# zju-vipa/ProtoPFormer

Measured on AMD Instinct MI355X. Metric: images/sec train step, deit_small+2000 protos, bs256, 1/2/4/8 MI355X, higher is better.
Workload: dtype bf16; 1 GPU; deit_small_patch16_224, synthetic 224x224, 2000x384 prototypes, 200 classes, k=81, batch 256/GPU (BASELINE.json configs[2]), train step = fwd+CE+PPC+bwd+allreduce+AdamW+EMA, DropPath 0.1; blocks after the token reservation run compacted on the 1+k reserved rows (equal to the masked full-length blocks to bf16 rounding); bf16 backbone: the reserved tokens differ from the fp32 reference's in ~2-3 % o; global_batch=256, parallelism=dp1

## Files before the change

protopformer_amd/csrc/gemm_bf16.hip:

```cpp
#include "ppf_common.h"
#include "ppf_hip.h"
#include "gemm_common.h"
#include "gemm_layout.h"
#include <cstdlib>
#include <type_traits>

namespace {
using namespace ppfg;

constexpr int BM = 128, BN = 128, NTHREADS = 256;
constexpr int TILE_BYTES = BM * BK * 2;
constexpr int STAGE_LD = 68;
constexpr int STAGE_BYTES = 4 * 32 * STAGE_LD * 4;


__device__ __forceinline__ int lds_off_mode0(int r, int c16) { return lds_row_off(r, c16); }

typedef uint32_t u32x4 __attribute__((ext_vector_type(4)));

template <bool T, int ROWS, int NTHR = NTHREADS>
struct TileIO {
    static constexpr int NLD = ROWS * 8 / NTHR;
    static constexpr int RPP = NTHR / 8;
    static constexpr int CPR = ROWS / 8;
    static constexpr int KPP = NTHR / CPR;
    static __device__ __forceinline__ unsigned gload(u32x4 (&reg)[NLD], const bf16_t* __restrict__ X, int ld, int R, int row0,
                                                     int k0, int kend, int tid, int kpad) {
        unsigned mask = 0;
        if constexpr (!T) {
            const int c16 = tid & 7, rb = tid >> 3;
            const bool kok = kpad ? (k0 + c16 * 8) < kend : (k0 + c16 * 8 + 8) <= kend;
            const int kk = kok ? k0 + c16 * 8 : 0;
#pragma unroll
            for (int i = 0; i < NLD; ++i) {
                const int r = row0 + rb + RPP * i;
                const bf16_t* src = X + (size_t)min(r, R - 1) * ld + kk;
                reg[i] = *reinterpret_cast<const u32x4*>(src);
                mask |= (kok && r < R) ? (1u << i) : 0u;
            }
        } else {
            const int c16 = tid % CPR, kb = tid / CPR;
            const int col = row0 + c16 * 8;
            const bool cok = kpad ? col < R : (col + 8) <= R;
            const int cc = cok ? col : 0;
#pragma unroll
            for (int i = 0; i < NLD; ++i) {
                const int kc = k0 + kb + KPP * i;
                const bf16_t* src = X + (size_t)min(kc, kend - 1) * ld + cc;
                reg[i] = *reinterpret_cast<const u32x4*>(src);
                mask |= (cok && kc < kend) ? (1u << i) : 0u;
            }
        }
        return mask;
    }
    static __device__ __forceinline__ void sstore(const u32x4 (&reg)[NLD], unsigned mask, unsigned char* tile, int tid) {
        const u32x4 zero = {0u, 0u, 0u, 0u};
        if constexpr (!T) {
            const int c16 = tid & 7, rb = tid >> 3;
#pragma unroll
            for (int i = 0; i < NLD; ++i)
                *reinterpret_cast<u32x4*>(tile + lds_off_mode0(rb + RPP * i, c16)) = ((mask >> i) & 1u) ? reg[i] : zero;
        } else {
            const int c16 = tid % CPR, kb = tid / CPR;
#pragma unroll
            for (int i = 0; i < NLD; ++i)
                *reinterpret_cast<u32x4*>(tile + lds_off_mode1<ROWS>(kb + KPP * i, c16 * 8)) = ((mask >> i) & 1u) ? reg[i] : zero;
        }
    }
    static __device__ __forceinline__ bf16x8 frag(const unsigned char* tile, int rbase, int ks, int lane) {
        if constexpr (!T) {
            return *reinterpret_cast<const bf16x8*>(tile + lds_off_mode0(rbase + (lane & 31), ks * 2 + (lane >> 5)));
        } else {
            typedef __attribute__((address_space(3))) bf16x4 lds_bf16x4;
            const int s = lane & 15, g16 = (lane >> 4) & 1, h = lane >> 5;
            const int col = rbase + 16 * g16 + 4 * (s & 3);
            const int kc = ks * 16 + 8 * h + (s >> 2);
            bf16x4 lo = __builtin_amdgcn_ds_read_tr16_b64_v4bf16((lds_bf16x4*)(tile + lds_off_mode1<ROWS>(kc, col)));
            bf16x4 hi = __builtin_amdgcn_ds_read_tr16_b64_v4bf16((lds_bf16x4*)(tile + lds_off_mode1<ROWS>(kc + 4, col)));
            return __builtin_shufflevector(lo, hi, 0, 1, 2, 3, 4, 5, 6, 7);
        }
    }
};


template <int EPI>
__device__ __forceinline__ void epilogue_rows(const GemmParams& p, const float* stage, int mbase, int nbase, int lane) {
    if (EpiWide<EPI>::value && ((p.ldc | p.ldaux) & 7) == 0) {
        const int col = (lane & 7) * 8;
        const int n = nbase + col;
        if (n + 8 <= p.N) {
            const EpiCols8 cc = epi_load_cols8<EPI>(p, n, true);
            EpiRow8 rr[4];
#pragma unroll
            for (int pass = 0; pass < 4; ++pass) {
                const int m = mbase + pass * 8 + (lane >> 3);
                rr[pass] = epi_load_row8<EPI>(p, m, n, m < p.M);
            }
#pragma unroll
            for (int pass = 0; pass < 4; ++pass) {
                const int r = pass * 8 + (lane >> 3);
                const int m = mbase + r;
                const float4 a = *reinterpret_cast<const float4*>(stage + r * STAGE_LD + col);
                const float4 b = *reinterpret_cast<const float4*>(stage + r * STAGE_LD + col + 4);
                if (m < p.M) epi_store8<EPI>(p, m, n, a, b, cc, rr[pass]);
            }
        } else if (n < p.N) {
            const EpiCols cc = epi_load_cols<EPI>(p, n, true);
#pragma unroll
            for (int pass = 0; pass < 4; ++pass) {
                const int r = pass * 8 + (lane >> 3);
                const int m = mbase + r;
                if (m < p.M) {
                    const EpiRow rr = epi_load_row<EPI>(p, m, n, true);
                    const float4 v = *reinterpret_cast<const float4*>(stage + r * STAGE_LD + col);
                    epi_store<EPI>(p, m, n, v.x, v.y, v.z, v.w, cc, rr);
                }
            }
        }
    } else {
        const int col = (lane & 15) * 4;
        const int n = nbase + col;
        const EpiCols cc = epi_load_cols<EPI>(p, n, n < p.N);
        EpiRow rr[8];
#pragma unroll
        for (int pass = 0; pass < 8; ++pass) {
            const int m = mbase + pass * 4 + (lane >> 4);
            rr[pass] = epi_load_row<EPI>(p, m, n, m < p.M && n < p.N);
        }
#pragma unroll
        for (int pass = 0; pass < 8; ++pass) {
            const int r = pass * 4 + (lane >> 4);
            const int m = mbase + r;
            const float4 v = *reinterpret_cast<const float4*>(stage + r * STAGE_LD + col);
            if (m < p.M && n < p.N) epi_store<EPI>(p, m, n, v.x, v.y, v.z, v.w, cc, rr[pass]);
        }
    }
}

template <int EPI, int MT>
__device__ __forceinline__ void strip_epilogue(const GemmParams& p, const f32x16 (&acc)[2][MT], int mi, unsigned char* smem, int wave, int lane,
                                               int mbase, int nbase) {
    const int h = lane >> 5;
    float* stage = reinterpret_cast<float*>(smem) + wave * (32 * STAGE_LD);
#pragma unroll
    for (int ni = 0; ni < 2; ++ni)
#pragma unroll
        for (int g = 0; g < 4; ++g)
            *reinterpret_cast<float4*>(stage + (lane & 31) * STAGE_LD + 32 * ni + 8 * g + 4 * h) =
                make_float4(acc[ni][mi][4 * g], acc[ni][mi][4 * g + 1], acc[ni][mi][4 * g + 2], acc[ni][mi][4 * g + 3]);
    __builtin_amdgcn_wave_barrier();
    epilogue_rows<EPI>(p, stage, mbase, nbase, lane);
    __builtin_amdgcn_wave_barrier();
}

__device__ __forceinline__ void store_partial_colsum(const GemmParams& p, int m, float v) {
    p.ws[p.zslice * ((size_t)p.M * p.N + (size_t)p.cs_parts * p.M) + (size_t)p.M * p.N + m] = v;
}

template <bool TA, bool TB, int EPI, bool COLSUM>
__global__ __launch_bounds__(NTHREADS, 3) void gemm_kernel(const GemmParams p_) {
    constexpr int PD = 1, MT = 2;
    extern __shared__ __attribute__((aligned(16))) unsigned char smem[];
    constexpr int TBM = 64 * MT;
    constexpr int A_BYTES = TBM * BK * 2;
    using IOA = TileIO<TA, TBM>;
    using IOB = TileIO<TB, BN>;
    const int tid = threadIdx.x, lane = tid & 63, wave = tid >> 6;
    const int wm = (wave & 1) * (32 * MT), wn = (wave >> 1) * 64;

    const int tiles_n = (p_.N + BN - 1) / BN;
    const int tiles = tiles_n * ((p_.M + TBM - 1) / TBM);
    const int vid_all = xcd_remap(blockIdx.x, gridDim.x);
    const int zslice = vid_all / tiles, vid = vid_all - zslice * tiles;
    const int m0 = (vid / tiles_n) * TBM, n0 = (vid % tiles_n) * BN;
    GemmParams p = p_;
    p.zslice = zslice;
    if (gridDim.y > 1) {
        const int bo = blockIdx.y / p.batch_inner, bi = blockIdx.y % p.batch_inner;
        p.A += bo * p.sa_o + bi * p.sa_i;
        p.B += bo * p.sb_o + bi * p.sb_i;
        const long long co = bo * p.sc_o + bi * p.sc_i;
        p.C = (EPI == EPI_BF16) ? (void*)(reinterpret_cast<bf16_t*>(p.C) + co) : (void*)(reinterpret_cast<float*>(p.C) + co);
    }

    const auto [kbeg, kend] = k_slice(p.K, p.nsplit, zslice);
    if (kbeg >= kend) return;
    const int nk = (kend - kbeg + BK - 1) / BK;

    u32x4 ra[PD][IOA::NLD], rb[PD][IOB::NLD];
    unsigned ma[PD], mb[PD];
    f32x16 acc[2][MT];
#pragma unroll
    for (int i = 0; i < 2; ++i)
#pragma unroll
        for (int j = 0; j < MT; ++j)
#pragma unroll
            for (int r = 0; r < 16; ++r) acc[i][j][r] = 0.f;
    f32x16 accs[MT];
    if constexpr (COLSUM) {
#pragma unroll
        for (int j = 0; j < MT; ++j)
#pragma unroll
            for (int r = 0; r < 16; ++r) accs[j][r] = 0.f;
    }
    const bool do_colsum = COLSUM && p.colsum != nullptr && n0 == 0 && wn == 0;
    unsigned char* tA = smem;
    unsigned char* tB = smem + A_BYTES;

#pragma unroll
    for (int st = 0; st < PD; ++st) {
        const int k0 = min(kbeg + st * BK, kbeg + (nk - 1) * BK);
        ma[st] = IOA::gload(ra[st], p.A, p.lda, p.M, m0, k0, kend, tid, p.kpad);
        mb[st] = IOB::gload(rb[st], p.B, p.ldb, p.N, n0, k0, kend, tid, p.kpad);
    }
    IOA::sstore(ra[0], ma[0], tA, tid);
    IOB::sstore(rb[0], mb[0], tB, tid);
    __syncthreads();

    for (int kt0 = 0; kt0 < nk; kt0 += PD) {
#pragma unroll
        for (int u = 0; u < PD; ++u) {
            const int kt = kt0 + u;
            if (kt >= nk) break;
            {
                const int k0 = kbeg + min(kt + PD, nk - 1) * BK;
                ma[u] = IOA::gload(ra[u], p.A, p.lda, p.M, m0, k0, kend, tid, p.kpad);
                mb[u] = IOB::gload(rb[u], p.B, p.ldb, p.N, n0, k0, kend, tid, p.kpad);
            }
#pragma unroll
            for (int ks = 0; ks < BK / 16; ++ks) {
                bf16x8 fa[MT], fb[2];
#pragma unroll
                for (int i = 0; i < MT; ++i) fa[i] = IOA::frag(tA, wm + 32 * i, ks, lane);
#pragma unroll
                for (int i = 0; i < 2; ++i) fb[i] = IOB::frag(tB, wn + 32 * i, ks, lane);
#pragma unroll
                for (int ni = 0; ni < 2; ++ni)
#pragma unroll
                    for (int mi = 0; mi < MT; ++mi)
                        acc[ni][mi] = __builtin_amdgcn_mfma_f32_32x32x16_bf16(fb[ni], fa[mi], acc[ni][mi], 0, 0, 0);
                if constexpr (COLSUM) {
                    if (do_colsum) {
                        bf16x8 ones;
#pragma unroll
                        for (int e = 0; e < 8; ++e) ones[e] = (__bf16)1.0f;
#pragma unroll
                        for (int mi = 0; mi < MT; ++mi)
                            accs[mi] = __builtin_amdgcn_mfma_f32_32x32x16_bf16(ones, fa[mi], accs[mi], 0, 0, 0);
                    }
                }
            }
            __syncthreads();
            if (kt + 1 < nk) {
                IOA::sstore(ra[(u + 1) % PD], ma[(u + 1) % PD], tA, tid);
                IOB::sstore(rb[(u + 1) % PD], mb[(u + 1) % PD], tB, tid);
            }
            __syncthreads();
        }
    }

#pragma unroll
    for (int mi = 0; mi < MT; ++mi) {
        strip_epilogue<EPI>(p, acc, mi, smem, wave, lane, m0 + wm + 32 * mi, n0 + wn);
        if constexpr (COLSUM) {
            const int m = m0 + wm + 32 * mi + (lane & 31);
            if (do_colsum && (lane >> 5) == 0 && m < p.M) {
                if constexpr (EPI == EPI_PARTIAL) store_partial_colsum(p, m, accs[mi][0]);
                else unsafeAtomicAdd(p.colsum + m, accs[mi][0]);
            }
        }
    }
}

#ifndef WG8_ISSUE_REGIONS
#define WG8_ISSUE_REGIONS 3
#endif
template <bool COLSUM>
__device__ __forceinline__ void wgrad8_mma(const bf16x8 (&fa)[2], const bf16x8 (&fb)[2], f32x16 (&acc)[2][2], f32x16 (&accs)[2], bool do_colsum) {
#pragma unroll
    for (int ni = 0; ni < 2; ++ni)
#pragma unroll
        for (int mi = 0; mi < 2; ++mi) acc[ni][mi] = __builtin_amdgcn_mfma_f32_32x32x16_bf16(fb[ni], fa[mi], acc[ni][mi], 0, 0, 0);
    if constexpr (COLSUM) {
        if (do_colsum) {
            bf16x8 ones;
#pragma unroll
            for (int e = 0; e < 8; ++e) ones[e] = (__bf16)1.0f;
#pragma unroll
            for (int mi = 0; mi < 2; ++mi) accs[mi] = __builtin_amdgcn_mfma_f32_32x32x16_bf16(ones, fa[mi], accs[mi], 0, 0, 0);
        }
    }
}

template <int WMW, int WNW, bool COLSUM, bool DMA>
__global__ __launch_bounds__(64 * WMW * WNW, 1) void wgrad8_kernel(const GemmParams p_) {
    extern __shared__ __attribute__((aligned(16))) unsigned char smem[];
    constexpr int NTHR = 64 * WMW * WNW, TBM = 64 * WMW, TBN = 64 * WNW;
    using IOA = TileIO<true, TBM, NTHR>;
    using IOB = TileIO<true, TBN, NTHR>;
    const int tid = threadIdx.x, lane = tid & 63;
    const int wave = __builtin_amdgcn_readfirstlane(tid >> 6);
    const int wm = (wave % WMW) * 64, wn = (wave / WMW) * 64;
    const int tiles_n = (p_.N + TBN - 1) / TBN;
    const int tiles = tiles_n * ((p_.M + TBM - 1) / TBM);
    const int vid_all = xcd_remap(blockIdx.x, gridDim.x);
    const int zslice = vid_all / tiles, vid = vid_all - zslice * tiles;
    const int m0 = (vid / tiles_n) * TBM, n0 = (vid % tiles_n) * TBN;
    GemmParams p = p_;
    p.zslice = zslice;
    const auto [kbeg, kend] = k_slice(p.K, p.nsplit, zslice);
    if (kbeg >= kend) return;
    const int nk = (kend - kbeg + BK - 1) / BK;

    f32x16 acc[2][2];
#pragma unroll
    for (int i = 0; i < 2; ++i)
#pragma unroll
        for (int j = 0; j < 2; ++j)
#pragma unroll
            for (int r = 0; r < 16; ++r) acc[i][j][r] = 0.f;
    f32x16 accs[2];
    if constexpr (COLSUM) {
#pragma unroll
        for (int j = 0; j < 2; ++j)
#pragma unroll
            for (int r = 0; r < 16; ++r) accs[j][r] = 0.f;
    }
    const bool do_colsum = COLSUM && p.colsum != nullptr && n0 == 0 && wn == 0;
    constexpr int A_BYTES = TBM * BK * 2;
    if constexpr (!DMA) {
        u32x4 ra[IOA::NLD], rb[IOB::NLD];
        unsigned ma, mb;
        unsigned char* tA = smem;
        unsigned char* tB = smem + A_BYTES;
        ma = IOA::gload(ra, p.A, p.lda, p.M, m0, kbeg, kend, tid, 0);
        mb = IOB::gload(rb, p.B, p.ldb, p.N, n0, kbeg, kend, tid, 0);
        IOA::sstore(ra, ma, tA, tid);
        IOB::sstore(rb, mb, tB, tid);
        __syncthreads();
        for (int kt = 0; kt < nk; ++kt) {
            {
                const int k0 = kbeg + min(kt + 1, nk - 1) * BK;
                ma = IOA::gload(ra, p.A, p.lda, p.M, m0, k0, kend, tid, 0);
                mb = IOB::gload(rb, p.B, p.ldb, p.N, n0, k0, kend, tid, 0);
            }
#pragma unroll
            for (int ks = 0; ks < BK / 16; ++ks) {
                bf16x8 fa[2], fb[2];
#pragma unroll
                for (int i = 0; i < 2; ++i) fa[i] = IOA::frag(tA, wm + 32 * i, ks, lane);
#pragma unroll
                for (int i = 0; i < 2; ++i) fb[i] = IOB::frag(tB, wn + 32 * i, ks, lane);
                wgrad8_mma<COLSUM>(fa, fb, acc, accs, do_colsum);
            }
            __syncthreads();
            if (kt + 1 < nk) {
                IOA::sstore(ra, ma, tA, tid);
                IOB::sstore(rb, mb, tB, tid);
            }
            __syncthreads();
        }
    } else {
        constexpr int NPA = TBM / 8, NPB = TBN / 8, PPW = (NPA + NPB) / 8;
        static_assert(NTHR == 512 && A_BYTES + TBN * BK * 2 == WG8_SLOT_BYTES && NPA % 8 == 0, "ring slot layout");
        const unsigned offA = (unsigned)(wgrad_dma_src(wgrad_dma_piece<TBM>(wave, lane), 0, p.lda, m0, p.M) * 2);
        const unsigned offB = (unsigned)(wgrad_dma_src(wgrad_dma_piece<TBN>(wave, lane), 0, p.ldb, n0, p.N) * 2);
        const size_t stepA = (size_t)p.lda * (BK * 2), stepB = (size_t)p.ldb * (BK * 2);
        const size_t pieceA = (size_t)p.lda * (4096 / TBM * 2), pieceB = (size_t)p.ldb * (4096 / TBN * 2);
        const unsigned char* gA = reinterpret_cast<const unsigned char*>(p.A) + (size_t)kbeg * p.lda * 2;
        const unsigned char* gB = reinterpret_cast<const unsigned char*>(p.B) + (size_t)kbeg * p.ldb * 2;
        const uint32_t ring = __builtin_amdgcn_readfirstlane(lds_offset_of(smem)) + wave * 1024;
        auto issue = [&](int i, uint32_t dst) __attribute__((always_inline)) {
            if (8 * i < NPA) lds_dma16_hidden(gA + i * pieceA + offA, dst + 8192 * i);
            else lds_dma16_hidden(gB + (i - NPA / 8) * pieceB + offB, dst + 8192 * i);
        };

        auto tile = [&](const unsigned char* st, uint32_t nxt, auto issue_tag) __attribute__((always_inline)) {
            constexpr bool ISSUE = decltype(issue_tag)::value;
            constexpr int NKS = BK / 16, NRI = WG8_ISSUE_REGIONS;
            const unsigned char* tA = st;
            const unsigned char* tB = st + A_BYTES;
            bf16x8 fa[2][2], fb[2][2];
#pragma unroll
            for (int i = 0; i < 2; ++i) fa[0][i] = IOA::frag(tA, wm + 32 * i, 0, lane);
#pragma unroll
            for (int i = 0; i < 2; ++i) fb[0][i] = IOB::frag(tB, wn + 32 * i, 0, lane);
#pragma unroll
            for (int ks = 0; ks < NKS; ++ks) {
                __builtin_amdgcn_sched_barrier(0);
                if constexpr (ISSUE) {
                    if (ks < NRI) {
#pragma unroll
                        for (int k = ks * PPW / NRI; k < (ks + 1) * PPW / NRI; ++k) issue(k, nxt);
                    }
                }
                if (ks + 1 < NKS) {
#pragma unroll
                    for (int i = 0; i < 2; ++i) fa[(ks + 1) & 1][i] = IOA::frag(tA, wm + 32 * i, ks + 1, lane);
#pragma unroll
                    for (int i = 0; i < 2; ++i) fb[(ks + 1) & 1][i] = IOB::frag(tB, wn + 32 * i, ks + 1, lane);
                }
                wgrad8_mma<COLSUM>(fa[ks & 1], fb[ks & 1], acc, accs, do_colsum);
            }
            __builtin_amdgcn_sched_barrier(0);
        };

#pragma unroll
        for (int i = 0; i < PPW; ++i) issue(i, ring);
        int slot = 0;
        for (int kt = 0; kt + 1 < nk; ++kt) {
            asm volatile("s_waitcnt vmcnt(0)" ::: "memory");
            __builtin_amdgcn_s_barrier();
            gA += stepA;
            gB += stepB;
            tile(smem + slot * WG8_SLOT_BYTES, ring + (slot ^ 1) * WG8_SLOT_BYTES, std::true_type());
            slot ^= 1;
        }
        asm volatile("s_waitcnt vmcnt(0)" ::: "memory");
        __builtin_amdgcn_s_barrier();
        tile(smem + slot * WG8_SLOT_BYTES, 0u, std::false_type());
        __syncthreads();
    }
#pragma unroll
    for (int mi = 0; mi < 2; ++mi) {
        strip_epilogue<EPI_PARTIAL>(p, acc, mi, smem, wave, lane, m0 + wm + 32 * mi, n0 + wn);
        if constexpr (COLSUM) {
            const int m = m0 + wm + 32 * mi + (lane & 31);
            if (do_colsum && (lane >> 5) == 0 && m < p.M) store_partial_colsum(p, m, accs[mi][0]);
        }
    }
}

int g_wgrad_path = 0;
#ifndef PPF_WGRAD_DMA_DEFAULT
#define PPF_WGRAD_DMA_DEFAULT 1
#endif
bool wgrad8_dma(const GemmParams& p) {
    if (p.K % BK != 0 || g_wgrad_path == 1) return false;
    return g_wgrad_path == 2 || PPF_WGRAD_DMA_DEFAULT;
}

template <int WMW, int WNW>
int launch_wgrad8(const GemmParams& p, int splitk, hipStream_t stream) {
    constexpr int NTHR = 64 * WMW * WNW, TBM = 64 * WMW, TBN = 64 * WNW;
    constexpr int opnd = (TBM + TBN) * BK * 2, strips = (NTHR / 64) * 32 * STAGE_LD * 4;
    constexpr int lds = opnd > strips ? opnd : strips;
    static_assert(strips <= WG8_RING_BYTES, "the epilogue strips reuse the dead ring");
    const int tiles = ((p.M + TBM - 1) / TBM) * ((p.N + TBN - 1) / TBN);
    if (wgrad8_dma(p)) return ppf_launch<wgrad8_kernel<WMW, WNW, true, true>>(dim3(tiles * splitk), dim3(NTHR), WG8_RING_BYTES, stream, "wgrad8 (dma)", p);
    return ppf_launch<wgrad8_kernel<WMW, WNW, true, false>>(dim3(tiles * splitk), dim3(NTHR), lds, stream, "wgrad8", p);
}

typedef __attribute__((address_space(3))) void g4_lds_t;
typedef const __attribute__((address_space(1))) void g4_gbl_t;

template <int NLA>
struct DirectLds {
    unsigned offA[NLA], offB[4];
    const unsigned char *gA, *gB;
    __device__ __forceinline__ DirectLds(const GemmParams& p, int m0, int n0, int tid)
        : gA(reinterpret_cast<const unsigned char*>(p.A)), gB(reinterpret_cast<const unsigned char*>(p.B)) {
        const int rb = tid >> 3, ch = (tid & 7) ^ lds_swz(rb);
#pragma unroll
        for (int i = 0; i < NLA; ++i) offA[i] = ((unsigned)min(m0 + rb + 32 * i, p.M - 1) * (unsigned)p.lda + ch * 8) * 2u;
#pragma unroll
        for (int i = 0; i < 4; ++i) offB[i] = ((unsigned)min(n0 + rb + 32 * i, p.N - 1) * (unsigned)p.ldb + ch * 8) * 2u;
    }
    __device__ __forceinline__ void load(int kt, unsigned char* tA, unsigned char* tB, int wave) const {
        const unsigned char* ka = gA + (size_t)kt * (BK * 2);
        const unsigned char* kb = gB + (size_t)kt * (BK * 2);
#pragma unroll
        for (int i = 0; i < NLA; ++i)
            __builtin_amdgcn_global_load_lds((g4_gbl_t*)(ka + offA[i]), (g4_lds_t*)(tA + i * 4096 + wave * 1024), 16, 0, 0);
#pragma unroll
        for (int i = 0; i < 4; ++i)
            __builtin_amdgcn_global_load_lds((g4_gbl_t*)(kb + offB[i]), (g4_lds_t*)(tB + i * 4096 + wave * 1024), 16, 0, 0);
        asm volatile("s_waitcnt vmcnt(0)" ::: "memory");
        __syncthreads();
    }
};

template <int EPI>
__global__ __launch_bounds__(NTHREADS, 4) void gemm128g_kernel(const GemmParams p) {
    extern __shared__ __attribute__((aligned(16))) unsigned char smem[];
    using IO = TileIO<false, 128>;
    const int tid = threadIdx.x, lane = tid & 63;
    const int wave = __builtin_amdgcn_readfirstlane(tid >> 6);
    const int wm = (wave & 1) * 64, wn = (wave >> 1) * 64;
    const int tiles_n = (p.N + BN - 1) / BN;
    const int vid = xcd_remap(blockIdx.x, gridDim.x);
    const int m0 = (vid / tiles_n) * BM, n0 = (vid % tiles_n) * BN;
    unsigned char* tA = smem;
    unsigned char* tB = smem + TILE_BYTES;
    const DirectLds<BM / 32> dl(p, m0, n0, tid);
    f32x16 acc[2][2];
#pragma unroll
    for (int i = 0; i < 2; ++i)
#pragma unroll
        for (int j = 0; j < 2; ++j)
#pragma unroll
            for (int r = 0; r < 16; ++r) acc[i][j][r] = 0.f;

    const int nk = p.K / BK;
    for (int kt = 0; kt < nk; ++kt) {
        if (kt > 0) __syncthreads();
        dl.load(kt, tA, tB, wave);
#pragma unroll
        for (int ks = 0; ks < BK / 16; ++ks) {
            bf16x8 fa[2], fb[2];
#pragma unroll
            for (int i = 0; i < 2; ++i) fa[i] = IO::frag(tA, wm + 32 * i, ks, lane);
#pragma unroll
            for (int i = 0; i < 2; ++i) fb[i] = IO::frag(tB, wn + 32 * i, ks, lane);
#pragma unroll
            for (int ni = 0; ni < 2; ++ni)
#pragma unroll
                for (int mi = 0; mi < 2; ++mi)
                    acc[ni][mi] = __builtin_amdgcn_mfma_f32_32x32x16_bf16(fb[ni], fa[mi], acc[ni][mi], 0, 0, 0);
        }
    }
    __syncthreads();
#pragma unroll
    for (int mi = 0; mi < 2; ++mi) strip_epilogue<EPI>(p, acc, mi, smem, wave, lane, m0 + wm + 32 * mi, n0 + wn);
}

template <int EPI>
int launch_g4(const GemmParams& p, hipStream_t stream) {
    constexpr int lds = 2 * TILE_BYTES > STAGE_BYTES ? 2 * TILE_BYTES : STAGE_BYTES;
    const int tiles = ((p.M + BM - 1) / BM) * ((p.N + BN - 1) / BN);
    return ppf_launch<gemm128g_kernel<EPI>>(dim3(tiles), dim3(NTHREADS), lds, stream, "gemm128g", p);
}

constexpr int G224_ROWS = 224, G224_MT = 7, G224_LD = 36;
__global__ __launch_bounds__(NTHREADS, 3) void gemm224g_kernel(const GemmParams p) {
    extern __shared__ __attribute__((aligned(16))) unsigned char smem[];
    using IO = TileIO<false, 128>;
    const int tid = threadIdx.x, lane = tid & 63;
    const int wave = __builtin_amdgcn_readfirstlane(tid >> 6);
    const int wn = wave * 32;
    const int tiles_n = (p.N + BN - 1) / BN;
    const int vid = xcd_remap(blockIdx.x, gridDim.x);
    const int m0 = (vid / tiles_n) * G224_ROWS, n0 = (vid % tiles_n) * BN;
    unsigned char* tA = smem;
    unsigned char* tB = smem + G224_ROWS * BK * 2;
    const DirectLds<G224_MT> dl(p, m0, n0, tid);
    f32x16 acc[G224_MT];
#pragma unroll
    for (int j = 0; j < G224_MT; ++j)
#pragma unroll
        for (int r = 0; r < 16; ++r) acc[j][r] = 0.f;
    const int nk = p.K / BK;
    for (int kt = 0; kt < nk; ++kt) {
        if (kt > 0) __syncthreads();
        dl.load(kt, tA, tB, wave);
#pragma unroll
        for (int ks = 0; ks < BK / 16; ++ks) {
            const bf16x8 fb = IO::frag(tB, wn, ks, lane);
#pragma unroll
            for (int mi = 0; mi < G224_MT; ++mi)
                acc[mi] = __builtin_amdgcn_mfma_f32_32x32x16_bf16(fb, IO::frag(tA, 32 * mi, ks, lane), acc[mi], 0, 0, 0);
        }
    }
    __syncthreads();
    const int h = lane >> 5;
    float* stage = reinterpret_cast<float*>(smem) + wave * (32 * G224_LD);
    bf16_t* C = reinterpret_cast<bf16_t*>(p.C);
#pragma unroll
    for (int mi = 0; mi < G224_MT; ++mi) {
#pragma unroll
        for (int g = 0; g < 4; ++g)
            *reinterpret_cast<float4*>(stage + (lane & 31) * G224_LD + 8 * g + 4 * h) =
                make_float4(acc[mi][4 * g], acc[mi][4 * g + 1], acc[mi][4 * g + 2], acc[mi][4 * g + 3]);
        __builtin_amdgcn_fence(__ATOMIC_RELEASE, "wavefront");
        __builtin_amdgcn_wave_barrier();
#pragma unroll
        for (int pass = 0; pass < 2; ++pass) {
            const int r = pass * 16 + (lane >> 2), col = (lane & 3) * 8;
            const int m = m0 + 32 * mi + r, n = n0 + wn + col;
            const float4 a = *reinterpret_cast<const float4*>(stage + r * G224_LD + col);
            const float4 b = *reinterpret_cast<const float4*>(stage + r * G224_LD + col + 4);
            if (m < p.M && n < p.N)
                *reinterpret_cast<uint4*>(C + (size_t)m * p.ldc + n) = make_uint4(pack_bf16x2(a.x * p.alpha, a.y * p.alpha), pack_bf16x2(a.z * p.alpha, a.w * p.alpha),
                                                                                 pack_bf16x2(b.x * p.alpha, b.y * p.alpha), pack_bf16x2(b.z * p.alpha, b.w * p.alpha));
        }
        __builtin_amdgcn_fence(__ATOMIC_RELEASE, "wavefront");
        __builtin_amdgcn_wave_barrier();
    }
}

bool g4_eligible(const GemmParams& p);
int g_force_g224 = 0;
bool g224_eligible(const GemmParams& p, int epi) {
    if (epi != EPI_BF16 || p.bias != nullptr || p.kpad || p.K % BK != 0 || p.N % 8 != 0 || (p.ldc & 7) != 0) return false;
    if ((long long)p.M * p.lda >= (1ll << 30) || (long long)p.N * p.ldb >= (1ll << 30)) return false;
    if (g_force_g224) return true;
    if (p.K < 768) return false;
    const int cus = ppf_cu_count();
    const long long tn = (p.N + BN - 1) / BN;
    const long long t128 = (long long)((p.M + BM - 1) / BM) * tn, t224 = (long long)((p.M + G224_ROWS - 1) / G224_ROWS) * tn;
    const int per128 = g4_eligible(p) ? 4 : 3;
    auto cost = [](long long tiles, long long slots, int rows, int per) {
        const long long full = tiles / slots, rest = tiles - full * slots;
        double c = (double)full * rows * per;
        if (rest) c += rows * per * (4 * rest >= slots ? 1.0 : 0.5);
        return c;
    };
    return t128 >= (long long)per128 * cus && cost(t224, 3ll * cus, G224_ROWS, 3) < 0.97 * cost(t128, (long long)per128 * cus, BM, per128);
}
int launch_g224(const GemmParams& p, hipStream_t stream) {
    constexpr int lds = G224_ROWS * BK * 2 + TILE_BYTES;
    const int tiles = ((p.M + G224_ROWS - 1) / G224_ROWS) * ((p.N + BN - 1) / BN);
    return ppf_launch<gemm224g_kernel>(dim3(tiles), dim3(NTHREADS), lds, stream, "gemm224g", p);
}

bool g4_eligible(const GemmParams& p) {
    return p.K % BK == 0 && p.K <= 512 && p.N >= 512 && !p.kpad && (long long)p.M * p.lda < (1ll << 30) &&
           (long long)p.N * p.ldb < (1ll << 30) && (long long)((p.M + BM - 1) / BM) * ((p.N + BN - 1) / BN) >= 512;
}

template <bool TA, bool TB, int EPI, bool COLSUM>
int launch(const GemmParams& p, int splitk, hipStream_t stream, int nbatch = 1) {
    const int tiles = ((p.M + BM - 1) / BM) * ((p.N + BN - 1) / BN);
    constexpr int lds = 2 * TILE_BYTES > STAGE_BYTES ? 2 * TILE_BYTES : STAGE_BYTES;
    GemmParams q = p;
    q.nsplit = splitk;
    return ppf_launch<gemm_kernel<TA, TB, EPI, COLSUM>>(dim3(tiles * splitk, nbatch, 1), dim3(NTHREADS), lds, stream, "gemm", q);
}

__global__ __launch_bounds__(256) void splitk_reduce_kernel(const float* __restrict__ ws, float* __restrict__ C, float* __restrict__ colsum,
                                                            int M, int N, int ldc, int nsplit, int cs_parts) {
    const size_t mn = (size_t)M * N, slice = mn + (colsum ? (size_t)cs_parts * M : 0);
    const size_t total4 = mn / 4;
    const size_t i = (size_t)blockIdx.x * 256 + threadIdx.x;
    if (i < total4) {
        const float* p = ws + i * 4;
        float4 acc = make_float4(0.f, 0.f, 0.f, 0.f);
        for (int z0 = 0; z0 < nsplit; z0 += 16) {
            float4 v[16];
#pragma unroll
            for (int u = 0; u < 16; ++u) {
                const int z = min(z0 + u, nsplit - 1);
                v[u] = *reinterpret_cast<const float4*>(p + (size_t)z * slice);
            }
#pragma unroll
            for (int u = 0; u < 16; ++u)
                if (z0 + u < nsplit) { acc.x += v[u].x; acc.y += v[u].y; acc.z += v[u].z; acc.w += v[u].w; }
        }
        const size_t e = i * 4, m = e / N, n = e - m * N;
        float4* dst = reinterpret_cast<float4*>(C + m * ldc + n);
        const float4 c = *dst;
        *dst = make_float4(c.x + acc.x, c.y + acc.y, c.z + acc.z, c.w + acc.w);
    } else if (colsum && i < total4 + (size_t)M) {
        const size_t m = i - total4;
        float a = 0.f;
        for (int z = 0; z < nsplit; ++z)
            for (int q = 0; q < cs_parts; ++q) a += ws[(size_t)z * slice + mn + (size_t)q * M + m];
        colsum[m] += a;
    }
}

PpfEventPool g_probe;
bool g_probe_on = false;

constexpr size_t PPF_GEMM_COUNTER_BYTES = 16384;


template <int... EPIS, class F>
bool dispatch_epi(int epi, int& rc, F&& f) {
    return ((epi == EPIS && (rc = f(std::integral_constant<int, EPIS>()), true)) || ...);
}

}

extern "C" {

int ppf_gemm_test_force_g224(int force) { g_force_g224 = force != 0; return 0; }

int ppf_gemm_test_wgrad_path(int path) {
    PPF_CHECK_ARG(path >= 0 && path <= 2, PPF_ERR_ARG, "ppf_gemm_test_wgrad_path: path must be 0, 1 or 2 (got %d)", path);
    g_wgrad_path = path;
    return 0;
}

size_t ppf_gemm_workspace_bytes(int M, int N, int K) {
    return PPF_GEMM_COUNTER_BYTES + (size_t)pick_splitk(M, N, K) * ((size_t)M * N + M) * sizeof(float);
}

int ppf_gemm_bf16(const void* A, const void* B, void* C, int M, int N, int K, int lda, int ldb, int ldc, int trans_a,
                  int trans_b, int epi, const float* bias, const float* res, int ldres, const float* rowscale,
                  int rows_per_group, const float* colscale, const void* aux_in, void* aux_out, int ldaux, float* colsum,
                  float alpha, void* workspace, size_t workspace_bytes, hipStream_t stream) {
    PPF_CHECK_ARG(M > 0 && N > 0 && K > 0, PPF_ERR_SHAPE, "ppf_gemm_bf16: bad shape M=%d N=%d K=%d", M, N, K);
    PPF_CHECK_ARG((lda % 8) == 0 && (ldb % 8) == 0 && (ldc % 4) == 0 && (N % 4) == 0, PPF_ERR_ALIGN,
                  "ppf_gemm_bf16: lda/ldb must be multiples of 8, ldc and N of 4 (lda=%d ldb=%d ldc=%d N=%d)", lda, ldb, ldc, N);
    PPF_CHECK_ARG(trans_a ? (M % 8 == 0) : (K % 8 == 0), PPF_ERR_ALIGN, "ppf_gemm_bf16: A inner extent must be a multiple of 8");
    PPF_CHECK_ARG(trans_b ? (N % 8 == 0) : (K % 8 == 0), PPF_ERR_ALIGN, "ppf_gemm_bf16: B inner extent must be a multiple of 8");
    PPF_CHECK_ARG((((uintptr_t)A | (uintptr_t)B | (uintptr_t)C) & 15) == 0, PPF_ERR_ALIGN, "ppf_gemm_bf16: pointers must be 16-byte aligned");
    PPF_CHECK_ARG(!(trans_a && !trans_b), PPF_ERR_ARG, "ppf_gemm_bf16: (trans_a=1, trans_b=0) is not instantiated");
    PPF_CHECK_ARG((((uintptr_t)aux_in | (uintptr_t)aux_out | (uintptr_t)res) & 15) == 0 && (ldaux % 4) == 0 && (ldres % 4) == 0, PPF_ERR_ALIGN,
                  "ppf_gemm_bf16: aux / residual pointers must be 16-byte aligned, ldaux and ldres multiples of 4 (the epilogues use 8/16-byte accesses)");
    GemmParams p;
    p.A = (const bf16_t*)A; p.B = (const bf16_t*)B; p.C = C; p.M = M; p.N = N; p.K = K; p.lda = lda; p.ldb = ldb; p.ldc = ldc;
    p.bias = bias; p.res = res; p.ldres = ldres; p.rowscale = rowscale; p.rows_per_group = rows_per_group > 0 ? rows_per_group : 1;
    p.colscale = colscale; p.aux_in = (const bf16_t*)aux_in; p.aux_out = (bf16_t*)aux_out; p.ldaux = ldaux; p.colsum = colsum; p.alpha = alpha; p.ws = nullptr;
    p.batch_inner = 1; p.sa_o = p.sa_i = p.sb_o = p.sb_i = p.sc_o = p.sc_i = 0; p.kpad = 0; p.cs_parts = 1; p.nsplit = 1;
    if (epi == EPI_RESID) PPF_CHECK_ARG(res != nullptr, PPF_ERR_ARG, "ppf_gemm_bf16: epi=4 needs a residual");
    if (epi == EPI_GELU) PPF_CHECK_ARG(aux_out != nullptr, PPF_ERR_ARG, "ppf_gemm_bf16: epi=2 needs aux_out");
    if (epi == EPI_DGELU) PPF_CHECK_ARG(aux_in != nullptr, PPF_ERR_ARG, "ppf_gemm_bf16: epi=5 needs aux_in");
    int rc;
    if (!trans_a && !trans_b) {
        if (g224_eligible(p, epi)) return launch_g224(p, stream);
        const auto g4 = [&](auto e) { return launch_g4<decltype(e)::value>(p, stream); };
        const auto nt = [&](auto e) { return launch<false, false, decltype(e)::value, false>(p, 1, stream); };
        if (g4_eligible(p) && dispatch_epi<EPI_BF16, EPI_GELU, EPI_RESID, EPI_DGELU>(epi, rc, g4)) return rc;
        if (dispatch_epi<EPI_BF16, EPI_F32, EPI_GELU, EPI_SIGMOID_F32, EPI_RESID, EPI_DGELU>(epi, rc, nt)) return rc;
    } else if (!trans_a && trans_b) {
        const auto nn = [&](auto e) { return launch<false, true, decltype(e)::value, false>(p, 1, stream); };
        if (dispatch_epi<EPI_BF16, EPI_F32, EPI_DGELU>(epi, rc, nn)) return rc;
    } else if (epi == EPI_ATOMIC) {
        const int ns = pick_splitk(M, N, K);
        const size_t need = PPF_GEMM_COUNTER_BYTES + (size_t)ns * ((size_t)M * N + M) * sizeof(float);
        if (workspace == nullptr || workspace_bytes < need || ns == 1) return launch<true, true, EPI_ATOMIC, true>(p, ns, stream);
        p.ws = (float*)((unsigned char*)workspace + PPF_GEMM_COUNTER_BYTES);
        p.cs_parts = 1;
        p.nsplit = ns;
        hipEvent_t e1 = nullptr;
        if (g_probe_on) {
            const auto ev = g_probe.acquire();
            (void)hipEventRecord(ev.first, stream);
            e1 = ev.second;
        }
        const bool wide = (M < N ? M : N) >= 320;
        if (wide && M >= 512 && M >= N && (M % 256 == 0 || M >= 1024)) rc = launch_wgrad8<4, 2>(p, ns, stream);
        else if (wide && N >= 512 && (N % 256 == 0 || N >= 1024)) rc = launch_wgrad8<2, 4>(p, ns, stream);
        else rc = launch<true, true, EPI_PARTIAL, true>(p, ns, stream);
        if (rc) return rc;
        if (e1) {
            (void)hipEventRecord(e1, stream);
            g_probe.flops += 2.0 * M * N * (double)K;
            g_probe.bytes += 2.0 * ((double)M * K + (double)N * K) + 4.0 * M * N;
        }
        const size_t work = (size_t)M * N / 4 + (colsum ? M : 0);
        const int grid = (int)((work + 255) / 256);
        hipLaunchKernelGGL(splitk_reduce_kernel, dim3(grid), dim3(256), 0, stream, p.ws, (float*)C, colsum, M, N, ldc, ns, p.cs_parts);
        PPF_LAUNCH_CHECK();
        return 0;
    } else if (epi == EPI_F32) {
        return launch<true, true, EPI_F32, false>(p, 1, stream);
    }
    ppf_set_error("ppf_gemm_bf16: combination trans_a=%d trans_b=%d epi=%d not instantiated", trans_a, trans_b, epi);
    return PPF_ERR_ARG;
}

int ppf_gemm_probe(int enable) {
    if (enable == 1) g_probe.reset();
    if (enable == 2) g_probe.destroy();
    g_probe_on = enable == 1;
    return 0;
}
int ppf_gemm_probe_read(double* ms_total, int64_t* launches, double* flops, double* bytes) {
    return g_probe.sum_ms("ppf_gemm_probe_read", ms_total, launches, flops, bytes);
}

int ppf_gemm_bf16_batched(const void* A, const void* B, void* C, int M, int N, int K, int lda, int ldb, int ldc, int trans_a, int trans_b,
                          int out_f32, float alpha, int batch_outer, int batch_inner, int64_t sa_o, int64_t sa_i, int64_t sb_o, int64_t sb_i,
                          int64_t sc_o, int64_t sc_i, int kpad, hipStream_t stream) {
    PPF_CHECK_ARG(M > 0 && N > 0 && K > 0 && batch_outer > 0 && batch_inner > 0, PPF_ERR_SHAPE, "ppf_gemm_bf16_batched: bad shape");
    PPF_CHECK_ARG((lda % 8) == 0 && (ldb % 8) == 0 && (ldc % 4) == 0 && (N % 4) == 0, PPF_ERR_ALIGN, "ppf_gemm_bf16_batched: ld alignment");
    PPF_CHECK_ARG(kpad || (trans_a ? (M % 8 == 0) : (K % 8 == 0)), PPF_ERR_ALIGN, "ppf_gemm_bf16_batched: A inner extent must be a multiple of 8");
    PPF_CHECK_ARG(kpad || (trans_b ? (N % 8 == 0) : (K % 8 == 0)), PPF_ERR_ALIGN, "ppf_gemm_bf16_batched: B inner extent must be a multiple of 8");
    PPF_CHECK_ARG(((sa_o | sa_i | sb_o | sb_i) % 8) == 0 && ((sc_o | sc_i) % 4) == 0, PPF_ERR_ALIGN, "ppf_gemm_bf16_batched: batch strides alignment");
    PPF_CHECK_ARG(out_f32 || (ldc % 8) != 0 || ((sc_o | sc_i) % 8) == 0, PPF_ERR_ALIGN,
                  "ppf_gemm_bf16_batched: bf16 output with ldc %% 8 == 0 needs batch strides of C that are multiples of 8 elements (sc_o=%lld sc_i=%lld)",
                  (long long)sc_o, (long long)sc_i);
    PPF_CHECK_ARG((((uintptr_t)A | (uintptr_t)B | (uintptr_t)C) & 15) == 0, PPF_ERR_ALIGN, "ppf_gemm_bf16_batched: pointers must be 16-byte aligned");
    GemmParams p;
    p.A = (const bf16_t*)A; p.B = (const bf16_t*)B; p.C = C; p.M = M; p.N = N; p.K = K; p.lda = lda; p.ldb = ldb; p.ldc = ldc;
    p.bias = nullptr; p.res = nullptr; p.ldres = 0; p.rowscale = nullptr; p.rows_per_group = 1; p.colscale = nullptr; p.aux_in = nullptr;
    p.aux_out = nullptr; p.ldaux = 0; p.colsum = nullptr; p.ws = nullptr; p.alpha = alpha;
    p.batch_inner = batch_inner; p.sa_o = sa_o; p.sa_i = sa_i; p.sb_o = sb_o; p.sb_i = sb_i; p.sc_o = sc_o; p.sc_i = sc_i; p.kpad = kpad;
    const int nb = batch_outer * batch_inner;
    const auto go = [&](auto ta, auto tb) {
        int rc = PPF_ERR_ARG;
        dispatch_epi<EPI_BF16, EPI_F32>(out_f32 ? EPI_F32 : EPI_BF16, rc, [&](auto e) {
            return launch<decltype(ta)::value, decltype(tb)::value, decltype(e)::value, false>(p, 1, stream, nb);
        });
        return rc;
    };
    if (!trans_a && !trans_b) return go(std::false_type(), std::false_type());
    if (!trans_a && trans_b) return go(std::false_type(), std::true_type());
    if (trans_a && trans_b) return go(std::true_type(), std::true_type());
    ppf_set_error("ppf_gemm_bf16_batched: (trans_a=1, trans_b=0) is not instantiated");
    return PPF_ERR_ARG;
}

}
```

protopformer_amd/csrc/gemm_common.h:

```cpp
#pragma once
#include "ppf_common.h"

namespace ppfg {

enum Epi { EPI_BF16 = 0, EPI_F32 = 1, EPI_GELU = 2, EPI_SIGMOID_F32 = 3, EPI_RESID = 4, EPI_DGELU = 5, EPI_ATOMIC = 6, EPI_PARTIAL = 7 };

struct GemmParams {
    const bf16_t* A; const bf16_t* B; void* C;
    int M, N, K, lda, ldb, ldc;
    const float* bias;
    const float* res;
    int ldres;
    const float* rowscale;
    int rows_per_group;
    const float* colscale;
    const bf16_t* aux_in;
    bf16_t* aux_out;
    int ldaux;
    float* colsum;
    float* ws;
    float alpha;
    int batch_inner;
    long long sa_o, sa_i, sb_o, sb_i, sc_o, sc_i;
    int zslice;
    int nsplit;
    int cs_parts;
    int kpad;
};

constexpr float GELU8_ZERO = 26.0f, GELU8_STEP = 1.0f / 196.0f, GELU8_INV = 196.0f;
__device__ __forceinline__ uint32_t gelu8_pack4(float a, float b, float c, float d) {
    uint32_t r = 0;
    r = __builtin_amdgcn_cvt_pk_u8_f32(a * GELU8_INV + GELU8_ZERO, 0, r);
    r = __builtin_amdgcn_cvt_pk_u8_f32(b * GELU8_INV + GELU8_ZERO, 1, r);
    r = __builtin_amdgcn_cvt_pk_u8_f32(c * GELU8_INV + GELU8_ZERO, 2, r);
    r = __builtin_amdgcn_cvt_pk_u8_f32(d * GELU8_INV + GELU8_ZERO, 3, r);
    return r;
}
__device__ __forceinline__ void gelu8_unpack4(uint32_t q, float (&d)[4]) {
    d[0] = ((float)(q & 0xffu) - GELU8_ZERO) * GELU8_STEP;
    d[1] = ((float)((q >> 8) & 0xffu) - GELU8_ZERO) * GELU8_STEP;
    d[2] = ((float)((q >> 16) & 0xffu) - GELU8_ZERO) * GELU8_STEP;
    d[3] = ((float)((q >> 24) & 0xffu) - GELU8_ZERO) * GELU8_STEP;
}

struct EpiCols { float4 bias, colscale; };
struct EpiRow { float4 res; uint2 aux; float rowscale; };

template <int EPI>
__device__ __forceinline__ EpiCols epi_load_cols(const GemmParams& p, int n0, bool ok) {
    EpiCols c;
    c.bias = make_float4(0.f, 0.f, 0.f, 0.f);
    c.colscale = make_float4(1.f, 1.f, 1.f, 1.f);
    if constexpr (EPI != EPI_ATOMIC && EPI != EPI_PARTIAL) {
        if (ok && p.bias) c.bias = *reinterpret_cast<const float4*>(p.bias + n0);
        if constexpr (EPI == EPI_RESID) { if (ok && p.colscale) c.colscale = *reinterpret_cast<const float4*>(p.colscale + n0); }
    }
    return c;
}

template <int EPI>
__device__ __forceinline__ EpiRow epi_load_row(const GemmParams& p, int m, int n0, bool ok) {
    EpiRow r;
    r.res = make_float4(0.f, 0.f, 0.f, 0.f); r.aux = make_uint2(0, 0); r.rowscale = 1.0f;
    if constexpr (EPI == EPI_RESID) {
        if (ok) {
            r.res = *reinterpret_cast<const float4*>(p.res + (size_t)m * p.ldres + n0);
            if (p.rowscale) r.rowscale = p.rowscale[m / p.rows_per_group];
        }
    } else if constexpr (EPI == EPI_DGELU) {
        if (ok) {
            const uint32_t t = __builtin_nontemporal_load(reinterpret_cast<const uint32_t*>(reinterpret_cast<const unsigned char*>(p.aux_in) + (size_t)m * p.ldaux + n0));
            r.aux = make_uint2(t, 0);
        }
    }
    return r;
}

template <int EPI>
__device__ __forceinline__ void epi_store(const GemmParams& p, int m, int n0, float v0, float v1, float v2, float v3, const EpiCols& cc, const EpiRow& rr) {
    float v[4] = {v0 * p.alpha, v1 * p.alpha, v2 * p.alpha, v3 * p.alpha};
    if constexpr (EPI == EPI_ATOMIC) {
        float* c = reinterpret_cast<float*>(p.C) + (size_t)m * p.ldc + n0;
#pragma unroll
        for (int i = 0; i < 4; ++i) unsafeAtomicAdd(c + i, v[i]);
        return;
    }
    if constexpr (EPI == EPI_PARTIAL) {
        const size_t slice = (size_t)p.M * p.N + (p.colsum ? (size_t)p.cs_parts * p.M : 0);
        float* dst = p.ws + p.zslice * slice + (size_t)m * p.N + n0;
        *reinterpret_cast<float4*>(dst) = make_float4(v[0], v[1], v[2], v[3]);
        return;
    }
    v[0] += cc.bias.x; v[1] += cc.bias.y; v[2] += cc.bias.z; v[3] += cc.bias.w;
    if constexpr (EPI == EPI_BF16) {
        *reinterpret_cast<uint2*>(reinterpret_cast<bf16_t*>(p.C) + (size_t)m * p.ldc + n0) =
            make_uint2(pack_bf16x2(v[0], v[1]), pack_bf16x2(v[2], v[3]));
    } else if constexpr (EPI == EPI_F32) {
        *reinterpret_cast<float4*>(reinterpret_cast<float*>(p.C) + (size_t)m * p.ldc + n0) = make_float4(v[0], v[1], v[2], v[3]);
    } else if constexpr (EPI == EPI_GELU) {
        ppf_float2 g01, d01, g23, d23;
        gelu_erf_both2(ppf_float2{v[0], v[1]}, g01, d01);
        gelu_erf_both2(ppf_float2{v[2], v[3]}, g23, d23);
        const float g[4] = {g01.x, g01.y, g23.x, g23.y}, d[4] = {d01.x, d01.y, d23.x, d23.y};
        __builtin_nontemporal_store(gelu8_pack4(d[0], d[1], d[2], d[3]), reinterpret_cast<uint32_t*>(reinterpret_cast<unsigned char*>(p.aux_out) + (size_t)m * p.ldaux + n0));
        *reinterpret_cast<uint2*>(reinterpret_cast<bf16_t*>(p.C) + (size_t)m * p.ldc + n0) = make_uint2(pack_bf16x2(g[0], g[1]), pack_bf16x2(g[2], g[3]));
    } else if constexpr (EPI == EPI_SIGMOID_F32) {
#pragma unroll
        for (int i = 0; i < 4; ++i) v[i] = 1.0f / (1.0f + __expf(-v[i]));
        *reinterpret_cast<float4*>(reinterpret_cast<float*>(p.C) + (size_t)m * p.ldc + n0) = make_float4(v[0], v[1], v[2], v[3]);
    } else if constexpr (EPI == EPI_RESID) {
        if (p.aux_out)
            *reinterpret_cast<uint2*>(p.aux_out + (size_t)m * p.ldaux + n0) = make_uint2(pack_bf16x2(v[0], v[1]), pack_bf16x2(v[2], v[3]));
        const float s = rr.rowscale;
        *reinterpret_cast<float4*>(reinterpret_cast<float*>(p.C) + (size_t)m * p.ldc + n0) =
            make_float4(rr.res.x + v[0] * cc.colscale.x * s, rr.res.y + v[1] * cc.colscale.y * s, rr.res.z + v[2] * cc.colscale.z * s,
                        rr.res.w + v[3] * cc.colscale.w * s);
    } else if constexpr (EPI == EPI_DGELU) {
        float hd[4];
        gelu8_unpack4(rr.aux.x, hd);
        *reinterpret_cast<uint2*>(reinterpret_cast<bf16_t*>(p.C) + (size_t)m * p.ldc + n0) =
            make_uint2(pack_bf16x2(v[0] * hd[0], v[1] * hd[1]), pack_bf16x2(v[2] * hd[2], v[3] * hd[3]));
    }
}

template <int EPI> struct EpiWide { static constexpr bool value = (EPI == EPI_BF16 || EPI == EPI_GELU || EPI == EPI_DGELU); };
struct EpiCols8 { float4 bias[2]; };
struct EpiRow8 { uint4 aux; };

template <int EPI>
__device__ __forceinline__ EpiCols8 epi_load_cols8(const GemmParams& p, int n0, bool ok) {
    EpiCols8 c;
    c.bias[0] = c.bias[1] = make_float4(0.f, 0.f, 0.f, 0.f);
    if (ok && p.bias) { c.bias[0] = *reinterpret_cast<const float4*>(p.bias + n0); c.bias[1] = *reinterpret_cast<const float4*>(p.bias + n0 + 4); }
    return c;
}
template <int EPI>
__device__ __forceinline__ EpiRow8 epi_load_row8(const GemmParams& p, int m, int n0, bool ok) {
    EpiRow8 r;
    r.aux = make_uint4(0, 0, 0, 0);
    if constexpr (EPI == EPI_DGELU) {
        if (ok) {
            typedef uint32_t u32x2 __attribute__((ext_vector_type(2)));
            const u32x2 t = __builtin_nontemporal_load(reinterpret_cast<const u32x2*>(reinterpret_cast<const unsigned char*>(p.aux_in) + (size_t)m * p.ldaux + n0));
            r.aux = make_uint4(t.x, t.y, 0, 0);
        }
    }
    return r;
}
template <int EPI>
__device__ __forceinline__ void epi_store8(const GemmParams& p, int m, int n0, const float4& a, const float4& b, const EpiCols8& cc, const EpiRow8& rr) {
    typedef uint32_t u32x4 __attribute__((ext_vector_type(4)));
    float v[8] = {a.x * p.alpha + cc.bias[0].x, a.y * p.alpha + cc.bias[0].y, a.z * p.alpha + cc.bias[0].z, a.w * p.alpha + cc.bias[0].w,
                  b.x * p.alpha + cc.bias[1].x, b.y * p.alpha + cc.bias[1].y, b.z * p.alpha + cc.bias[1].z, b.w * p.alpha + cc.bias[1].w};
    bf16_t* dst = reinterpret_cast<bf16_t*>(p.C) + (size_t)m * p.ldc + n0;
    if constexpr (EPI == EPI_BF16) {
        *reinterpret_cast<uint4*>(dst) = make_uint4(pack_bf16x2(v[0], v[1]), pack_bf16x2(v[2], v[3]), pack_bf16x2(v[4], v[5]), pack_bf16x2(v[6], v[7]));
    } else if constexpr (EPI == EPI_GELU) {
        ppf_float2 g[4], d[4];
#pragma unroll
        for (int i = 0; i < 4; ++i) gelu_erf_both2(ppf_float2{v[2 * i], v[2 * i + 1]}, g[i], d[i]);
        typedef uint32_t u32x2 __attribute__((ext_vector_type(2)));
        const u32x2 dv = {gelu8_pack4(d[0].x, d[0].y, d[1].x, d[1].y), gelu8_pack4(d[2].x, d[2].y, d[3].x, d[3].y)};
        __builtin_nontemporal_store(dv, reinterpret_cast<u32x2*>(reinterpret_cast<unsigned char*>(p.aux_out) + (size_t)m * p.ldaux + n0));
        *reinterpret_cast<uint4*>(dst) = make_uint4(pack_bf16x2(g[0].x, g[0].y), pack_bf16x2(g[1].x, g[1].y), pack_bf16x2(g[2].x, g[2].y), pack_bf16x2(g[3].x, g[3].y));
    } else if constexpr (EPI == EPI_DGELU) {
        float ha[4], hb[4];
        gelu8_unpack4(rr.aux.x, ha);
        gelu8_unpack4(rr.aux.y, hb);
        *reinterpret_cast<uint4*>(dst) = make_uint4(pack_bf16x2(v[0] * ha[0], v[1] * ha[1]), pack_bf16x2(v[2] * ha[2], v[3] * ha[3]),
                                                    pack_bf16x2(v[4] * hb[0], v[5] * hb[1]), pack_bf16x2(v[6] * hb[2], v[7] * hb[3]));
    }
}


}
```

Baseline: 17340 images/sec.

## Hoist GEMM epilogue operand loads ahead of per-strip epilogue with optional prefetch

```diff
diff --git a/protopformer_amd/csrc/gemm_bf16.hip b/protopformer_amd/csrc/gemm_bf16.hip
--- a/protopformer_amd/csrc/gemm_bf16.hip
+++ b/protopformer_amd/csrc/gemm_bf16.hip
@@ -83,35 +83,107 @@
 };
 
 
+#ifndef PPF_EPI_PREFETCH
+#define PPF_EPI_PREFETCH 0
+#endif
 template <int EPI>
-__device__ __forceinline__ void epilogue_rows(const GemmParams& p, const float* stage, int mbase, int nbase, int lane) {
-    if (EpiWide<EPI>::value && ((p.ldc | p.ldaux) & 7) == 0) {
+__device__ __forceinline__ bool epi_wide(const GemmParams& p) { return EpiWide<EPI>::value && ((p.ldc | p.ldaux) & 7) == 0; }
+
+template <int EPI, int MT>
+__device__ __forceinline__ void epi_fetch(const GemmParams& p, EpiOperands<EPI>& o, int mbase, int nbase, int lane) {
+    static_assert(MT <= 2, "EpiOperands holds the row operands of two blocks");
+    float4 c0 = make_float4(0.f, 0.f, 0.f, 0.f), c1 = make_float4(1.f, 1.f, 1.f, 1.f);
+    uint32_t a[2][8] = {{0, 0, 0, 0, 0, 0, 0, 0}, {0, 0, 0, 0, 0, 0, 0, 0}};
+    if constexpr (EpiHasOperands<EPI>::value) {
+        if (epi_wide<EPI>(p)) {
+            const int n = nbase + (lane & 7) * 8;
+            if (n + 8 <= p.N) {
+                const EpiCols8 c = epi_load_cols8<EPI>(p, n, true);
+                c0 = c.bias[0]; c1 = c.bias[1];
+                if constexpr (EPI == EPI_DGELU) {
+#pragma unroll
+                    for (int mi = 0; mi < MT; ++mi)
+#pragma unroll
+                        for (int pass = 0; pass < 4; ++pass) {
+                            const int m = mbase + 32 * mi + pass * 8 + (lane >> 3);
+                            const EpiRow8 r = epi_load_row8<EPI>(p, m, n, m < p.M);
+                            a[mi][2 * pass] = r.aux.x; a[mi][2 * pass + 1] = r.aux.y;
+                        }
+                }
+            } else if (n < p.N) {
+                const EpiCols c = epi_load_cols<EPI>(p, n, true);
+                c0 = c.bias; c1 = c.colscale;
+                if constexpr (EPI == EPI_DGELU) {
+#pragma unroll
+                    for (int mi = 0; mi < MT; ++mi)
+#pragma unroll
+                        for (int pass = 0; pass < 4; ++pass) {
+                            const int m = mbase + 32 * mi + pass * 8 + (lane >> 3);
+                            a[mi][pass] = epi_load_row<EPI>(p, m, n, m < p.M).aux.x;
+                        }
+                }
+            }
+        } else {
+            const int n = nbase + (lane & 15) * 4;
+            const EpiCols c = epi_load_cols<EPI>(p, n, n < p.N);
+            c0 = c.bias; c1 = c.colscale;
+            if constexpr (EPI == EPI_DGELU) {
+#pragma unroll
+                for (int mi = 0; mi < MT; ++mi)
+#pragma unroll
+                    for (int pass = 0; pass < 8; ++pass) {
+                        const int m = mbase + 32 * mi + pass * 4 + (lane >> 4);
+                        a[mi][pass] = epi_load_row<EPI>(p, m, n, m < p.M && n < p.N).aux.x;
+                    }
+            }
+        }
+    }
+    o.c0 = c0; o.c1 = c1;
+    if constexpr (EPI == EPI_DGELU) {
+#pragma unroll
+        for (int mi = 0; mi < 2; ++mi)
+#pragma unroll
+            for (int i = 0; i < 8; ++i) o.aux[mi][i] = a[mi][i];
+    }
+}
+
+template <int EPI>
+__device__ __forceinline__ EpiRow epi_row4(const GemmParams& p, const EpiOperands<EPI>& o, int blk, int pass, int m, int n, bool ok) {
+    if constexpr (EPI == EPI_RESID) return epi_load_row<EPI>(p, m, n, ok);
+    EpiRow r;
+    r.res = make_float4(0.f, 0.f, 0.f, 0.f); r.aux = make_uint2(0, 0); r.rowscale = 1.0f;
+    if constexpr (EPI == EPI_DGELU) r.aux.x = o.aux[blk][pass];
+    return r;
+}
+
+template <int EPI>
+__device__ __forceinline__ void epilogue_finish(const GemmParams& p, const EpiOperands<EPI>& o, int blk, const float* stage, int mbase, int nbase, int lane) {
+    if (epi_wide<EPI>(p)) {
         const int col = (lane & 7) * 8;
         const int n = nbase + col;
         if (n + 8 <= p.N) {
-            const EpiCols8 cc = epi_load_cols8<EPI>(p, n, true);
-            EpiRow8 rr[4];
-#pragma unroll
-            for (int pass = 0; pass < 4; ++pass) {
-                const int m = mbase + pass * 8 + (lane >> 3);
-                rr[pass] = epi_load_row8<EPI>(p, m, n, m < p.M);
-            }
+            EpiCols8 cc;
+            cc.bias[0] = o.c0; cc.bias[1] = o.c1;
 #pragma unroll
             for (int pass = 0; pass < 4; ++pass) {
                 const int r = pass * 8 + (lane >> 3);
                 const int m = mbase + r;
+                EpiRow8 rr;
+                rr.aux = make_uint4(0, 0, 0, 0);
+                if constexpr (EPI == EPI_DGELU) { rr.aux.x = o.aux[blk][2 * pass]; rr.aux.y = o.aux[blk][2 * pass + 1]; }
                 const float4 a = *reinterpret_cast<const float4*>(stage + r * STAGE_LD + col);
                 const float4 b = *reinterpret_cast<const float4*>(stage + r * STAGE_LD + col + 4);
-                if (m < p.M) epi_store8<EPI>(p, m, n, a, b, cc, rr[pass]);
+                if (m < p.M) epi_store8<EPI>(p, m, n, a, b, cc, rr);
             }
         } else if (n < p.N) {
-            const EpiCols cc = epi_load_cols<EPI>(p, n, true);
+            EpiCols cc;
+            cc.bias = o.c0; cc.colscale = o.c1;
 #pragma unroll
             for (int pass = 0; pass < 4; ++pass) {
                 const int r = pass * 8 + (lane >> 3);
                 const int m = mbase + r;
                 if (m < p.M) {
-                    const EpiRow rr = epi_load_row<EPI>(p, m, n, true);
+                    const EpiRow rr = epi_row4<EPI>(p, o, blk, pass, m, n, true);
                     const float4 v = *reinterpret_cast<const float4*>(stage + r * STAGE_LD + col);
                     epi_store<EPI>(p, m, n, v.x, v.y, v.z, v.w, cc, rr);
                 }
@@ -120,13 +192,15 @@
     } else {
         const int col = (lane & 15) * 4;
         const int n = nbase + col;
-        const EpiCols cc = epi_load_cols<EPI>(p, n, n < p.N);
+        EpiCols cc;
+        cc.bias = o.c0; cc.colscale = o.c1;
         EpiRow rr[8];
 #pragma unroll
         for (int pass = 0; pass < 8; ++pass) {
             const int m = mbase + pass * 4 + (lane >> 4);
-            rr[pass] = epi_load_row<EPI>(p, m, n, m < p.M && n < p.N);
-        }
+            rr[pass] = epi_row4<EPI>(p, o, blk, pass, m, n, m < p.M && n < p.N);
+        }
+        if constexpr (EPI == EPI_RESID) epi_operands_wait();
 #pragma unroll
         for (int pass = 0; pass < 8; ++pass) {
             const int r = pass * 4 + (lane >> 4);
@@ -139,7 +213,7 @@
 
 template <int EPI, int MT>
 __device__ __forceinline__ void strip_epilogue(const GemmParams& p, const f32x16 (&acc)[2][MT], int mi, unsigned char* smem, int wave, int lane,
-                                               int mbase, int nbase) {
+                                               int mbase, int nbase, const EpiOperands<EPI>& o) {
     const int h = lane >> 5;
     float* stage = reinterpret_cast<float*>(smem) + wave * (32 * STAGE_LD);
 #pragma unroll
@@ -149,7 +223,7 @@
             *reinterpret_cast<float4*>(stage + (lane & 31) * STAGE_LD + 32 * ni + 8 * g + 4 * h) =
                 make_float4(acc[ni][mi][4 * g], acc[ni][mi][4 * g + 1], acc[ni][mi][4 * g + 2], acc[ni][mi][4 * g + 3]);
     __builtin_amdgcn_wave_barrier();
-    epilogue_rows<EPI>(p, stage, mbase, nbase, lane);
+    epilogue_finish<EPI>(p, o, mi, stage, mbase, nbase, lane);
     __builtin_amdgcn_wave_barrier();
 }
 
@@ -259,9 +333,12 @@
         }
     }
 
+    EpiOperands<EPI> eo;
+    epi_fetch<EPI, MT>(p, eo, m0 + wm, n0 + wn, lane);
+    if constexpr (EpiHasOperands<EPI>::value) epi_operands_wait();
 #pragma unroll
     for (int mi = 0; mi < MT; ++mi) {
-        strip_epilogue<EPI>(p, acc, mi, smem, wave, lane, m0 + wm + 32 * mi, n0 + wn);
+        strip_epilogue<EPI>(p, acc, mi, smem, wave, lane, m0 + wm + 32 * mi, n0 + wn, eo);
         if constexpr (COLSUM) {
             const int m = m0 + wm + 32 * mi + (lane & 31);
             if (do_colsum && (lane >> 5) == 0 && m < p.M) {
@@ -421,9 +498,11 @@
         tile(smem + slot * WG8_SLOT_BYTES, 0u, std::false_type());
         __syncthreads();
     }
+    EpiOperands<EPI_PARTIAL> eo;
+    epi_fetch<EPI_PARTIAL, 2>(p, eo, m0 + wm, n0 + wn, lane);
 #pragma unroll
     for (int mi = 0; mi < 2; ++mi) {
-        strip_epilogue<EPI_PARTIAL>(p, acc, mi, smem, wave, lane, m0 + wm + 32 * mi, n0 + wn);
+        strip_epilogue<EPI_PARTIAL>(p, acc, mi, smem, wave, lane, m0 + wm + 32 * mi, n0 + wn, eo);
         if constexpr (COLSUM) {
             const int m = m0 + wm + 32 * mi + (lane & 31);
             if (do_colsum && (lane >> 5) == 0 && m < p.M) store_partial_colsum(p, m, accs[mi][0]);
@@ -501,27 +580,39 @@
 #pragma unroll
             for (int r = 0; r < 16; ++r) acc[i][j][r] = 0.f;
 
+    auto mma_tile = [&]() __attribute__((always_inline)) {
+#pragma unroll
+        for (int ks = 0; ks < BK / 16; ++ks) {
+            bf16x8 fa[2], fb[2];
+#pragma unroll
+            for (int i = 0; i < 2; ++i) fa[i] = IO::frag(tA, wm + 32 * i, ks, lane);
+#pragma unroll
+            for (int i = 0; i < 2; ++i) fb[i] = IO::frag(tB, wn + 32 * i, ks, lane);
+#pragma unroll
+            for (int ni = 0; ni < 2; ++ni)
+#pragma unroll
+                for (int mi = 0; mi < 2; ++mi)
+                    acc[ni][mi] = __builtin_amdgcn_mfma_f32_32x32x16_bf16(fb[ni], fa[mi], acc[ni][mi], 0, 0, 0);
+        }
+    };
     const int nk = p.K / BK;
-    for (int kt = 0; kt < nk; ++kt) {
+    for (int kt = 0; kt + 1 < nk; ++kt) {
         if (kt > 0) __syncthreads();
         dl.load(kt, tA, tB, wave);
-#pragma unroll
-        for (int ks = 0; ks < BK / 16; ++ks) {
-            bf16x8 fa[2], fb[2];
-#pragma unroll
-            for (int i = 0; i < 2; ++i) fa[i] = IO::frag(tA, wm + 32 * i, ks, lane);
-#pragma unroll
-            for (int i = 0; i < 2; ++i) fb[i] = IO::frag(tB, wn + 32 * i, ks, lane);
-#pragma unroll
-            for (int ni = 0; ni < 2; ++ni)
-#pragma unroll
-                for (int mi = 0; mi < 2; ++mi)
-                    acc[ni][mi] = __builtin_amdgcn_mfma_f32_32x32x16_bf16(fb[ni], fa[mi], acc[ni][mi], 0, 0, 0);
-        }
-    }
+        mma_tile();
+    }
+    if (nk > 1) __syncthreads();
+    dl.load(nk - 1, tA, tB, wave);
+    EpiOperands<EPI> eo;
+    if constexpr (PPF_EPI_PREFETCH) epi_fetch<EPI, 2>(p, eo, m0 + wm, n0 + wn, lane);
+    __builtin_amdgcn_sched_barrier(0);
+    mma_tile();
+    __builtin_amdgcn_sched_barrier(0);
     __syncthreads();
-#pragma unroll
-    for (int mi = 0; mi < 2; ++mi) strip_epilogue<EPI>(p, acc, mi, smem, wave, lane, m0 + wm + 32 * mi, n0 + wn);
+    if constexpr (!PPF_EPI_PREFETCH) epi_fetch<EPI, 2>(p, eo, m0 + wm, n0 + wn, lane);
+    epi_operands_wait();
+#pragma unroll
+    for (int mi = 0; mi < 2; ++mi) strip_epilogue<EPI>(p, acc, mi, smem, wave, lane, m0 + wm + 32 * mi, n0 + wn, eo);
 }
 
 template <int EPI>
diff --git a/protopformer_amd/csrc/gemm_common.h b/protopformer_amd/csrc/gemm_common.h
--- a/protopformer_amd/csrc/gemm_common.h
+++ b/protopformer_amd/csrc/gemm_common.h
@@ -173,5 +173,13 @@
     }
 }
 
+template <int EPI>
+struct EpiOperands {
+    float4 c0, c1;
+    uint32_t aux[2][8];
+};
+template <int EPI> struct EpiHasOperands { static constexpr bool value = (EPI != EPI_ATOMIC && EPI != EPI_PARTIAL); };
+
+__device__ __forceinline__ void epi_operands_wait() { __builtin_amdgcn_s_waitcnt(0x0F70); }
 
 }
```

Result: no change. 17330 images/sec (-0.1%).
